# zengyan-97/X2-VLM

Hardware: AMD Instinct MI355X
Metric: image-text pairs/sec (fwd+bwd) X2VLM-base 224px bs=64/GPU (higher is better)
Workload: dtype bf16

## Files before the change

### include/x2vlm_hip.h

```cpp
#ifndef X2VLM_HIP_H
#define X2VLM_HIP_H
#include <stdint.h>
#ifdef __cplusplus
extern "C" {
#endif

const char* x2_last_error(void);
int x2_abi_version(void);
int x2_device_cus(void);
int x2_tune(int key, int value);
int x2_tune_get(int key);

int x2_gemm_nt(const void* A, const void* B, void* C, int M, int N, int K, int lda, int ldb, int ldc,
               const float* bias, const float* gamma, const float* resid, int ldr, void* aux, int ldaux,
               int act, int out_f32, unsigned drop_thr16, unsigned drop_seed, float drop_scale, const unsigned* drop_epoch,
               const float* rowscale, float* colsum, void* stream);

int x2_gemm_nt_dgelu_colparts(const void* A, const void* B, void* C, int M, int N, int K, int lda, int ldb, int ldc,
                              const void* aux, int ldaux, float* colparts, int* nrows_out, void* stream);
int x2_gemm_nt_splitk(const void* A, const void* B, float* C, int M, int N, int K, int lda, int ldb, int ldc,
                      int slices, float* ws, long ws_floats, void* stream);

int x2_gemm_tn_grouped(const int64_t* problems, int count, int accumulate, int split, float* ws, long ws_floats,
                       void* stream);

typedef struct X2AttnArgs {
  const void *Q, *K, *V, *O, *dO;
  void *Out, *dQ, *dK, *dV, *dS;
  float *LSE, *Delta;
  long q_bs, q_rs, k_bs, k_rs, v_bs, v_rs, o_bs, o_rs;
  long dq_bs, dq_rs, dk_bs, dk_rs, dv_bs, dv_rs, do_bs, do_rs;
  int B, Bkv, H, Lq, Lk;
  float scale;
  const float* bias;  int bias_ld;
  const float* biasT; int biasT_ld;
  const float* mask;  int mask_ld;
  const int* kv_idx;
  const int* seq_off; const int* seq_ids;
  int ds_ld;
  unsigned drop_thr16, drop_seed; float drop_scale;
  int dbg;
  int head_dim;
  const unsigned* drop_epoch;
  int grid_nx, grid_ny, grid_nz, grid_map;
  int phase;
  float* ws; long ws_floats;
  float* colsum_ws;
} X2AttnArgs;
int x2_attn_fwd(const X2AttnArgs* args, void* stream);
int x2_attn_bwd(const X2AttnArgs* args, void* stream);
int x2_attn_bwd_one_pass(const X2AttnArgs* args);

int x2_layernorm_fwd(const float* x, const float* w, const float* b, void* y_bf16, float* y_f32, float* mean,
                     float* rstd, int rows, int D, float eps, int period, unsigned drop_thr16, unsigned drop_seed,
                     float drop_scale, const unsigned* drop_epoch, void* stream);
int x2_layernorm_bwd(const void* dy , int dy_is_bf16, const float* x, const float* mean, const float* rstd, const float* w,
                     const float* dres, float* dx, void* dx_bf16, float* dw, float* db, float* dcol, int rows, int D,
// ... 129 lines not shown
```

### x2-vlm_amd/_lib.py

```python
import contextlib
import ctypes as C
import os

import torch

_HERE = os.path.dirname(os.path.abspath(__file__))
LIB_PATH = os.environ.get("X2VLM_HIP_LIB") or os.path.join(_HERE, "libx2vlm_hip.so")

P, I, L, F, U = C.c_void_p, C.c_int, C.c_long, C.c_float, C.c_uint


class AttnArgs(C.Structure):
    _fields_ = [(n, P) for n in ("Q", "K", "V", "O", "dO", "Out", "dQ", "dK", "dV", "dS", "LSE", "Delta")] + \
               [(n, L) for n in ("q_bs", "q_rs", "k_bs", "k_rs", "v_bs", "v_rs", "o_bs", "o_rs",
                                 "dq_bs", "dq_rs", "dk_bs", "dk_rs", "dv_bs", "dv_rs", "do_bs", "do_rs")] + \
               [(n, I) for n in ("B", "Bkv", "H", "Lq", "Lk")] + [("scale", F)] + \
               [("bias", P), ("bias_ld", I), ("biasT", P), ("biasT_ld", I), ("mask", P), ("mask_ld", I),
                ("kv_idx", P), ("seq_off", P), ("seq_ids", P), ("ds_ld", I),
                ("drop_thr16", C.c_uint), ("drop_seed", C.c_uint), ("drop_scale", F), ("dbg", I), ("head_dim", I), ("drop_epoch", P),
                ("grid_nx", I), ("grid_ny", I), ("grid_nz", I), ("grid_map", I),
                ("phase", I), ("ws", P), ("ws_floats", L), ("colsum_ws", P)]


_SIGS = {
    "x2_gemm_nt": [P, P, P, I, I, I, I, I, I, P, P, P, I, P, I, I, I, U, U, F, P, P, P, P],
    "x2_gemm_nt_splitk": [P, P, P, I, I, I, I, I, I, I, P, L, P],
    "x2_gemm_nt_dgelu_colparts": [P, P, P, I, I, I, I, I, I, P, I, P, C.POINTER(I), P],
    "x2_gemm_tn_grouped": [P, I, I, I, P, L, P],
    "x2_attn_fwd": [C.POINTER(AttnArgs), P],
    "x2_attn_bwd": [C.POINTER(AttnArgs), P],
    "x2_layernorm_fwd": [P, P, P, P, P, P, P, I, I, F, I, U, U, F, P, P],
    "x2_layernorm_bwd": [P, I, P, P, P, P, P, P, P, P, P, P, I, I, I, U, U, F, U, U, F, P, P, I, I, P, P],
    "x2_colsum_bf16": [P, P, I, I, I, P, I, P],
    "x2_reduce_partials": [P, I, I, I, P, P, P, P],
    "x2_reduce_partials_multi": [P, I, P],
    "x2_cast_transpose_multi": [P, I, P],
    "x2_copy_f32_multi": [P, I, P],
    "x2_layerscale_finish": [P, I, P],
    "x2_rowscale_cast_colsum": [P, P, P, P, I, I, P, I, P],
    "x2_cast_bf16": [P, P, L, P],
    "x2_cast_transpose_bf16": [P, P, P, I, I, I, P],
    "x2_patchify": [P, P, I, I, I, P],
    "x2_assemble_tokens": [P, P, P, I, I, I, P],
    "x2_assemble_tokens_bwd": [P, P, P, I, I, I, P],
    "x2_pool_tokens": [P, P, I, I, I, I, P],
    "x2_relpos_bias": [P, P, P, P, P, I, I, I, I, F, P],
    "x2_relpos_bias_bwd": [P, P, P, P, I, I, I, I, I, P, I, P],
    "x2_embed_fwd": [P, P, P, P, P, I, I, I, P],
    "x2_embed_bwd": [P, P, P, P, P, I, I, I, P, P],
    "x2_gather_rows": [P, P, P, P, I, L, P],
    "x2_scatter_rows": [P, P, P, I, I, L, P],
    "x2_linear_f32": [P, P, P, P, P, F, I, I, I, L, L, L, L, L, I, I, P, P],
    "x2_l2norm": [P, P, P, I, I, I, P],
    "x2_ce_fwd": [P, L, P, I, I, P, P, P, P],
    "x2_ce_bwd": [P, L, P, P, P, P, F, I, I, P, P, L, P],
    "x2_mlm_ce_fwd": [P, P, P, P, I, I, I, I, I, I, P, P, P],
    "x2_ce_combine": [P, I, P, P, I, P, P, P, P],
    "x2_mlm_ce_bwd": [P, P, P, P, P, P, P, F, I, I, I, I, I, I, P, L, P],
    "x2_sample_negatives": [P, I, P, P, P, P],
    "x2_mask_tokens": [P, P, I, I, P, I, P, I, U, P, C.c_double, I, C.c_double, I, I, L, L, L, L, P, P, P, P],
    "x2_additive_mask": [P, P, I, I, I, F, P],
# ... 13 lines not shown
    "x2_mlm_ls_fwd": [P, P, P, P, L, I, I, I, I, I, I, P, P, P, P, P],
    "x2_ls_combine": [P, P, I, P, P, P, P, I, I, L, F, P, P, P, P],
    "x2_mlm_ls_bwd": [P, P, P, P, P, P, P, P, F, F, L, I, I, I, I, I, I, P, L, P],
    "x2_attn_decode": [P, I, P, P, I, I, I, I, I, I, F, P],
    "x2_beam_gather": [P, P, P, I, I, I, I, I, P],
    "x2_logprob_topk": [P, I, I, I, P, I, I, I, I, I, I, P, P, P, P],
    "x2_answer_topk": [P, I, I, I, P, I, I, P, P, P],
    "x2_vqa_candidates": [P, P, P, I, I, I, I, L, P, P, P, P, I, P],
    "x2_vqa_rerank": [P, I, P, P, I, I, P, P, P, P],
    "x2_bbox_loss_fwd": [P, P, P, I, P, P, P],
    "x2_bbox_loss_bwd": [P, P, P, P, P, P, P, I, P, P],
    "x2_grounding_iou": [P, P, P, I, P, P, P],
    "x2_cls_tail_fwd": [P, I, P, P, P, P, P, I, I, I, F, P, P, P, P, P],
    "x2_cls_tail_bwd": [P, I, P, P, P, P, P, P, P, P, P, I, I, I, P, I, P, P, P, P, P],
    "x2_cls_accuracy": [P, P, I, I, P, P, P],
    "x2_lngelu_fwd": [P, I, P, P, I, I, F, P, I, P, P],
    "x2_lngelu_bwd": [P, I, P, I, P, P, P, I, I, P, I, P, P, P],
    "x2_soft_ce_fwd": [P, I, I, I, P, P, P, I, P, P, P, P],
    "x2_kl_ce_fwd": [P, I, P, I, I, I, P, P, P, P, P],
    "x2_soft_ce_bwd": [P, I, I, I, P, P, P, P, P, P, P, I, P, I, I, P],
    "x2_kl_ce_bwd": [P, I, P, I, I, I, P, P, P, P, I, P, I, I, P],
    "x2_cls_accuracy_rows": [P, I, P, I, I, P, P, P, P],
}
_COMM_SIGS = {
    "x2_comm_unique_id": [P],
    "x2_comm_init": [P, I, I, C.POINTER(P)],
    "x2_comm_info": [P, C.POINTER(I), C.POINTER(I)],
    "x2_comm_allreduce_bucket": [P, P, L, I, I, P, P],
    "x2_comm_allgather": [P, P, P, L, I, P, P],
    "x2_comm_broadcast": [P, P, L, I, I, P, P],
    "x2_comm_destroy": [P],
}
EXPORTS = sorted(list(_SIGS) + list(_COMM_SIGS) + ["x2_last_error", "x2_abi_version", "x2_device_cus", "x2_tune", "x2_tune_get",
                                                         "x2_attn_bwd_one_pass"])

_lib = None


class X2HipError(RuntimeError):
    pass


def lib():
    global _lib
    if _lib is None:
        if not os.path.exists(LIB_PATH):
            raise X2HipError("HIP extension %s not built: run `python -c 'import __graft_entry__ as g; g.build()'`"
                             % LIB_PATH)
        try:
            h = C.CDLL(LIB_PATH)
        except OSError as e:
            raise X2HipError("cannot load %s: %s" % (LIB_PATH, e))
        for name, sig in list(_SIGS.items()) + list(_COMM_SIGS.items()):
            fn = getattr(h, name)
            fn.argtypes, fn.restype = sig, I
        h.x2_last_error.restype = C.c_char_p
        h.x2_abi_version.restype = I
        h.x2_device_cus.restype = I
        h.x2_tune.argtypes, h.x2_tune.restype = [I, I], I
        h.x2_tune_get.argtypes, h.x2_tune_get.restype = [I], I
        h.x2_attn_bwd_one_pass.argtypes, h.x2_attn_bwd_one_pass.restype = [C.POINTER(AttnArgs)], I
        for kv in filter(None, os.environ.get("X2_TUNE", "").split(",")):
            k, v = kv.split("=")
            set_tune(int(k), int(v), h)
        _lib = h
    return _lib


def set_tune(key, value, h=None):
    h = lib() if h is None else h
    if h.x2_tune(key, value) != 0:
        raise X2HipError("x2_tune(%d, %d): %s" % (key, value, h.x2_last_error().decode()))


@contextlib.contextmanager
def tuned(knobs):
    h = lib()
    with contextlib.ExitStack() as undo:
        for key, value in knobs.items():
            prev = h.x2_tune_get(key)
            if prev == -1:
                raise X2HipError("x2_tune_get(%d): no such key" % key)
            if prev != value:
                set_tune(key, value, h)
                undo.callback(set_tune, key, prev, h)
        yield


_get_device = torch._C._cuda_getDevice if hasattr(torch._C, "_cuda_getDevice") else None
_get_raw_stream = getattr(torch._C, "_cuda_getCurrentRawStream", None)


def raw_stream():
    return _get_raw_stream(_get_device())
# ... 12 lines not shown
```

### x2-vlm_amd/csrc/gemm.hip

```cpp
#include "x2_common.h"
#include <type_traits>

#define BM 128
#define BN 128
#define BK 64
#define TILE_BYTES (128 * 128)
#define STAGE_BYTES (2 * TILE_BYTES)
#define GEMM_LDS_BYTES (2 * STAGE_BYTES)

struct GemmNT {
  const bf16_t* A; const bf16_t* B; void* C;
  const float* bias; const float* gamma; const float* resid; bf16_t* aux;
  int M, N, K;
  int lda, ldb, ldc, ldr, ldaux;
  int act;
  int out_f32;
  int group_m;
  DropSpec drop;
  const uint32_t* drop_epoch;
  const float* rowscale;
  float* colsum;
  int dbg;
  int ksplit;
  const long* ce_labels;
  const float* ce_lse;
  const float* ce_g;
  const float* ce_stat;
  float* ce_part;
  float* ce_zlab;
  float ce_gscale;
  int ce_C;
  float* ce_sumz;
  float* ce_zign;
  long ce_ignore;
// ... 1163 lines not shown
  launch_nt_ce(p, 9, (hipStream_t)stream);
  return x2_check_launch("x2_mlm_ce_bwd");
}
extern "C" int x2_mlm_ls_fwd(const void* X, const void* E, const float* bias, const long* labels, long ignore, int R, int Vp, int V, int Hd,
                             int ldx, int lde, float* part, float* sumz, float* zlab, float* zign, void* stream) {
  X2_REQUIRE(X && E && labels && part && sumz && zlab && zign, "x2_mlm_ls_fwd: null argument");
  X2_REQUIRE(mlm_ce_shapes_ok(R, Vp, V, Hd, ldx, lde) && V > 2 && ignore >= 0 && ignore < V,
             "x2_mlm_ls_fwd: R=%d Vp=%d V=%d Hd=%d ldx=%d lde=%d ignore=%ld", R, Vp, V, Hd, ldx, lde, ignore);
  GemmNT p{(const bf16_t*)X, (const bf16_t*)E, nullptr, bias, nullptr, nullptr, nullptr, R, Vp, Hd, ldx, lde, Vp, 0, 0, 0, 0,
           g_tune[0] > 0 ? g_tune[0] : 8, DropSpec{0u, 0u, 1.f}, nullptr, nullptr, nullptr, 0, 0,
           labels, nullptr, nullptr, nullptr, part, zlab, 1.f, V, sumz, zign, ignore, 0.f, nullptr};
  launch_nt_ce(p, 11, (hipStream_t)stream);
  return x2_check_launch("x2_mlm_ls_fwd");
}
extern "C" int x2_mlm_ls_bwd(const void* X, const void* E, const float* bias, const long* labels, const float* w, const float* lse, const float* g,
                             const float* stat, float gscale, float ls, long ignore, int R, int Vp, int V, int Hd, int ldx, int lde, void* dl_bf16,
                             long ldd, void* stream) {
  X2_REQUIRE(X && E && labels && w && lse && g && stat && dl_bf16, "x2_mlm_ls_bwd: null argument");
  X2_REQUIRE(mlm_ce_shapes_ok(R, Vp, V, Hd, ldx, lde) && ldd >= Vp && ldd % 8 == 0 && V > 2 && ignore >= 0 && ignore < V && ls >= 0.f && ls <= 1.f,
             "x2_mlm_ls_bwd: R=%d Vp=%d V=%d Hd=%d ldd=%ld ignore=%ld", R, Vp, V, Hd, ldd, ignore);
  GemmNT p{(const bf16_t*)X, (const bf16_t*)E, dl_bf16, bias, nullptr, nullptr, nullptr, R, Vp, Hd, ldx, lde, (int)ldd, 0, 0, 0, 0,
           g_tune[0] > 0 ? g_tune[0] : 8, DropSpec{0u, 0u, 1.f}, nullptr, nullptr, nullptr, 0, 0,
           labels, lse, g, stat, nullptr, nullptr, gscale, V, nullptr, nullptr, ignore, ls, w};
  launch_nt_ce(p, 12, (hipStream_t)stream);
  return x2_check_launch("x2_mlm_ls_bwd");
}

struct TNProblem {
  const bf16_t* A; const bf16_t* B; float* C;
  int Mc, N, K;
  int lda, ldb, ldc;
  int n_ld, k_ld;
  int tile_begin, tiles_k;
};
struct GemmTNGroup { TNProblem p[8]; int count; int accumulate; };

__device__ __forceinline__ int tn_f(int r) { return (r & 3) | (((r >> 3) & 1) << 2); }

__global__ __launch_bounds__(256, 2) void gemm_tn_kernel(GemmTNGroup g) {
  extern __shared__ __attribute__((aligned(16))) char smem[];
  const int tid = threadIdx.x, lane = tid & 63;
  const int wave = __builtin_amdgcn_readfirstlane(tid >> 6);
  const int wn = wave >> 1, wk = wave & 1;
  int t = xcd_remap(blockIdx.x, gridDim.x);
  int pi = 0;
#pragma unroll
  for (int i = 1; i < 8; ++i) if (i < g.count && t >= g.p[i].tile_begin) pi = i;
  const TNProblem p = g.p[pi];
  t -= p.tile_begin;
  int tnn, tkk;
  tile_coords(t, (p.N + 127) / 128, p.tiles_k, 8, tnn, tkk);
  const int n0 = tnn * 128, k0 = tkk * 128;
  const int steps = (p.Mc + BK - 1) / BK;
  const int per = (steps + gridDim.y - 1) / gridDim.y;
  const int s_begin = blockIdx.y * per, s_end = min(steps, s_begin + per);
  if (s_begin >= s_end) return;

  const bf16_t* srcA[4]; const bf16_t* srcB[4]; int rowq[4];
#pragma unroll
  for (int i = 0; i < 4; ++i) {
    const int q = i * 256 + tid, row = q >> 4, c = (q & 15) ^ (tn_f(row) << 1);
    int ca = n0 + c * 8; ca = ca <= p.n_ld - 8 ? ca : p.n_ld - 8;
    int cb = k0 + c * 8; cb = cb <= p.k_ld - 8 ? cb : p.k_ld - 8;
    rowq[i] = row;
    srcA[i] = p.A + (size_t)row * p.lda + ca;
    srcB[i] = p.B + (size_t)row * p.ldb + cb;
  }
  auto stage = [&](int s, int buf) {
    char* base = smem + buf * STAGE_BYTES;
    const int mbase = s * BK;
    if (mbase + BK <= p.Mc) {
#pragma unroll
      for (int i = 0; i < 4; ++i) {
        glds16(srcA[i] + (size_t)mbase * p.lda, base + (i * 256 + wave * 64) * 16);
        glds16(srcB[i] + (size_t)mbase * p.ldb, base + TILE_BYTES + (i * 256 + wave * 64) * 16);
      }
    } else {
#pragma unroll
      for (int i = 0; i < 4; ++i) {
        u32x4 va = u32x4{0, 0, 0, 0}, vb = u32x4{0, 0, 0, 0};
        if (mbase + rowq[i] < p.Mc) {
          va = *reinterpret_cast<const u32x4*>(srcA[i] + (size_t)mbase * p.lda);
// ... 52 lines not shown
    const int n = n0 + wn * 64 + j * 16 + fi;
    if (n >= p.N) continue;
#pragma unroll
    for (int i = 0; i < 4; ++i) {
      const int k = k0 + wk * 64 + i * 16 + fg * 4;
      if (k >= p.K) continue;
      float* dst = p.C + (size_t)n * p.ldc + k;
      if (atomic) {
#pragma unroll
        for (int r = 0; r < 4; ++r) atomicAdd(dst + r, acc[i][j][r]);
      } else if (g.accumulate) {
        float4 o = *reinterpret_cast<float4*>(dst);
        o.x += acc[i][j][0]; o.y += acc[i][j][1]; o.z += acc[i][j][2]; o.w += acc[i][j][3];
        *reinterpret_cast<float4*>(dst) = o;
      } else {
        *reinterpret_cast<float4*>(dst) = float4{acc[i][j][0], acc[i][j][1], acc[i][j][2], acc[i][j][3]};
      }
    }
  }
}

#define T2_HALF 16384
#define T2_LDS_BYTES (8 * T2_HALF)
__device__ __attribute__((aligned(16))) const uint32_t x2_zero_chunk[4] = {0u, 0u, 0u, 0u};
template <bool RAG>
__global__ __launch_bounds__(512) void gemm_tn256_kernel(GemmTNGroup g, float* ws, int total_tiles) {
  extern __shared__ __attribute__((aligned(16))) char smem[];
  const int tid = threadIdx.x, lane = tid & 63;
  const int wave = __builtin_amdgcn_readfirstlane(tid >> 6);
  const int wr = wave >> 2, wc = wave & 3;
  const int tile = xcd_remap(blockIdx.x, gridDim.x);
  int pi = 0;
#pragma unroll
  for (int i = 1; i < 8; ++i) if (i < g.count && tile >= g.p[i].tile_begin) pi = i;
  const TNProblem p = g.p[pi];
  int tnn, tkk;
  tile_coords(tile - p.tile_begin, (p.N + 255) / 256, p.tiles_k, 4, tnn, tkk);
  const int n0 = tnn * 256, k0 = tkk * 256;
  const int steps = (p.Mc + BK - 1) / BK, rag = p.Mc % BK;
  const int s_begin = (int)((long)steps * blockIdx.y / gridDim.y), s_end = (int)((long)steps * (blockIdx.y + 1) / gridDim.y);
  const int nk = s_end - s_begin;
  const int last_rel = (RAG && rag != 0 && s_end == steps) ? nk - 1 : -1;
  const bf16_t* const zsrc = reinterpret_cast<const bf16_t*>(x2_zero_chunk);
  const bool oob0 = (tid >> 4) >= rag, oob1 = ((512 + tid) >> 4) >= rag;

  const bf16_t* srcA[2][2]; const bf16_t* srcB[2][2];
#pragma unroll
  for (int h = 0; h < 2; ++h)
#pragma unroll
    for (int i = 0; i < 2; ++i) {
      const int q = i * 512 + tid, row = q >> 4, c = (q & 15) ^ (tn_f(row) << 1);
      int ca = n0 + h * 128 + c * 8; ca = ca <= p.n_ld - 8 ? ca : p.n_ld - 8;
      int cb = k0 + h * 128 + c * 8; cb = cb <= p.k_ld - 8 ? cb : p.k_ld - 8;
      srcA[h][i] = p.A + ((size_t)s_begin * BK + row) * p.lda + ca;
      srcB[h][i] = p.B + ((size_t)s_begin * BK + row) * p.ldb + cb;
    }
  const size_t stepA = (size_t)BK * p.lda, stepB = (size_t)BK * p.ldb;
  auto issue = [&](int kt, auto slot) {
    constexpr int S = decltype(slot)::value;
    char* base = smem + ((kt & 1) * 4 + S) * T2_HALF + wave * 1024;
    const bool z = RAG && kt == last_rel;
    if constexpr (S < 2) {
      glds16(z && oob0 ? zsrc : srcA[S][0] + kt * stepA, base);
      glds16(z && oob1 ? zsrc : srcA[S][1] + kt * stepA, base + 8192);
    } else {
      glds16(z && oob0 ? zsrc : srcB[S - 2][0] + kt * stepB, base);
      glds16(z && oob1 ? zsrc : srcB[S - 2][1] + kt * stepB, base + 8192);
    }
  };
  using S0 = std::integral_constant<int, 0>; using S1 = std::integral_constant<int, 1>;
// ... 68 lines not shown
  int kt = 0;
  for (; kt + 2 < nk; ++kt) ktile(kt, std::true_type{}, std::true_type{});
  if (kt + 1 < nk) { ktile(kt, std::true_type{}, std::false_type{}); ++kt; }
  ktile(kt, std::false_type{}, std::false_type{});

  if (gridDim.y > 1) {
    float* dst = ws + ((size_t)blockIdx.y * total_tiles + tile) * 65536 + (size_t)wave * 8192 + lane * 4;
#pragma unroll
    for (int i = 0; i < 4; ++i)
#pragma unroll
      for (int j = 0; j < 8; ++j)
        *reinterpret_cast<float4*>(dst + (i * 8 + j) * 256) = float4{acc[i][j][0], acc[i][j][1], acc[i][j][2], acc[i][j][3]};
    return;
  }
#pragma unroll
  for (int j = 0; j < 8; ++j) {
    const int n = n0 + wr * 128 + j * 16 + fi;
    if (n >= p.N) continue;
#pragma unroll
    for (int i = 0; i < 4; ++i) {
      const int k = k0 + wc * 64 + i * 16 + fg * 4;
      if (k >= p.K) continue;
      float* dst = p.C + (size_t)n * p.ldc + k;
      float4 o = float4{acc[i][j][0], acc[i][j][1], acc[i][j][2], acc[i][j][3]};
      if (g.accumulate) { const float4 c = *reinterpret_cast<float4*>(dst); o.x += c.x; o.y += c.y; o.z += c.z; o.w += c.w; }
      *reinterpret_cast<float4*>(dst) = o;
    }
  }
}
__global__ __launch_bounds__(256) void gemm_tn256_reduce_kernel(GemmTNGroup g, const float* __restrict__ ws, int total_tiles, int split) {
  const int tile = blockIdx.x >> 6;
  int pi = 0;
#pragma unroll
  for (int i = 1; i < 8; ++i) if (i < g.count && tile >= g.p[i].tile_begin) pi = i;
  const TNProblem p = g.p[pi];
  int tnn, tkk;
  tile_coords(tile - p.tile_begin, (p.N + 255) / 256, p.tiles_k, 4, tnn, tkk);
  const int e = (blockIdx.x & 63) * 256 + threadIdx.x;
  const int lane = e & 63, ij = (e >> 6) & 31, wave = e >> 11;
  const int i = ij >> 3, j = ij & 7, fi = lane & 15, fg = lane >> 4, wr = wave >> 2, wc = wave & 3;
  const int n = tnn * 256 + wr * 128 + j * 16 + fi, k = tkk * 256 + wc * 64 + i * 16 + fg * 4;
  const float* src = ws + (size_t)tile * 65536 + (size_t)e * 4;
  float4 o = *reinterpret_cast<const float4*>(src);
  for (int s_ = 1; s_ < split; ++s_) {
    const float4 v = *reinterpret_cast<const float4*>(src + (size_t)s_ * total_tiles * 65536);
    o.x += v.x; o.y += v.y; o.z += v.z; o.w += v.w;
  }
  if (n >= p.N || k >= p.K) return;
  float* dst = p.C + (size_t)n * p.ldc + k;
  if (g.accumulate) { const float4 c = *reinterpret_cast<float4*>(dst); o.x += c.x; o.y += c.y; o.z += c.z; o.w += c.w; }
  *reinterpret_cast<float4*>(dst) = o;
}

extern "C" int x2_gemm_tn_grouped(const int64_t* problems, int count, int accumulate, int split, float* ws, long ws_floats,
                                  void* stream) {
  X2_REQUIRE(count >= 1 && count <= 8, "x2_gemm_tn_grouped: count=%d not in [1,8]", count);
  X2_REQUIRE(split >= 0, "x2_gemm_tn_grouped: split=%d", split);
  GemmTNGroup g; g.count = count; g.accumulate = accumulate;
  int tiles = 0, tiles256 = 0, min_steps = 1 << 30;
  bool big = g_tune[5] != 1;
  for (int i = 0; i < count; ++i) {
    const int64_t* q = problems + i * 11;
    TNProblem& p = g.p[i];
    p.A = (const bf16_t*)q[0]; p.B = (const bf16_t*)q[1]; p.C = (float*)q[2];
    p.Mc = (int)q[3]; p.N = (int)q[4]; p.K = (int)q[5]; p.lda = (int)q[6]; p.ldb = (int)q[7]; p.ldc = (int)q[8];
    p.n_ld = (int)q[9]; p.k_ld = (int)q[10];
    X2_REQUIRE(p.Mc > 0 && p.N > 0 && p.K > 0, "x2_gemm_tn_grouped[%d]: empty problem", i);
    X2_REQUIRE(p.K % 4 == 0 && p.ldc % 4 == 0, "x2_gemm_tn_grouped[%d]: K, ldc must be multiples of 4", i);
    X2_REQUIRE(p.lda % 8 == 0 && p.ldb % 8 == 0 && p.n_ld % 8 == 0 && p.k_ld % 8 == 0 && p.n_ld >= 8 && p.k_ld >= 8,
               "x2_gemm_tn_grouped[%d]: rows must be 16-byte granular", i);
    X2_REQUIRE(p.n_ld <= p.lda && p.k_ld <= p.ldb, "x2_gemm_tn_grouped[%d]: n_ld/k_ld exceed leading dims", i);
    tiles += ((p.N + 127) / 128) * ((p.K + 127) / 128);
    tiles256 += ((p.N + 255) / 256) * ((p.K + 255) / 256);
    const int steps_i = (p.Mc + BK - 1) / BK;
    min_steps = steps_i < min_steps ? steps_i : min_steps;
  }
  if (g_tune[5] != 2 && tiles256 < 24 && !(split > 1 && ws)) big = false;
  if (big) {
    int t = 0;
    for (int i = 0; i < count; ++i) { g.p[i].tile_begin = t; g.p[i].tiles_k = (g.p[i].K + 255) / 256; t += ((g.p[i].N + 255) / 256) * g.p[i].tiles_k; }
    const int cus = x2_cus();
    int sp = split;
    if (sp == 0) {
      double best = -1.0; sp = 1;
      for (int c = 1; c <= 4 && min_steps / c >= 16; ++c) {
        const long blocks = (long)t * c;
        const double fill = (double)blocks / (double)(((blocks + cus - 1) / cus) * cus);
        if (fill > best + 0.03) { best = fill; sp = c; }
      }
    }
    while (sp > 1 && (sp > min_steps || !ws || (long)sp * t * 65536 > ws_floats)) --sp;
    static bool attr = false;
    if (!attr) {
      (void)hipFuncSetAttribute(reinterpret_cast<const void*>(gemm_tn256_kernel<false>), hipFuncAttributeMaxDynamicSharedMemorySize, T2_LDS_BYTES);
      (void)hipFuncSetAttribute(reinterpret_cast<const void*>(gemm_tn256_kernel<true>), hipFuncAttributeMaxDynamicSharedMemorySize, T2_LDS_BYTES);
      attr = true;
    }
    bool ragged = false;
    for (int i = 0; i < count; ++i) ragged = ragged || (g.p[i].Mc % BK != 0);
    if (ragged) hipLaunchKernelGGL(gemm_tn256_kernel<true>, dim3(t, sp), dim3(512), T2_LDS_BYTES, (hipStream_t)stream, g, ws, t);
    else hipLaunchKernelGGL(gemm_tn256_kernel<false>, dim3(t, sp), dim3(512), T2_LDS_BYTES, (hipStream_t)stream, g, ws, t);
    if (sp > 1) hipLaunchKernelGGL(gemm_tn256_reduce_kernel, dim3(t * 64), dim3(256), 0, (hipStream_t)stream, g, ws, t, sp);
    return x2_check_launch("x2_gemm_tn_grouped");
  }
  if (split == 0) split = 1;
  X2_REQUIRE(split == 1 || accumulate, "x2_gemm_tn_grouped: split>1 on the 128x128 kernel adds atomically: pass accumulate=1 and a defined C");
  int t = 0;
  for (int i = 0; i < count; ++i) { g.p[i].tile_begin = t; g.p[i].tiles_k = (g.p[i].K + 127) / 128; t += ((g.p[i].N + 127) / 128) * g.p[i].tiles_k; }
  hipLaunchKernelGGL(gemm_tn_kernel, dim3(t, split), dim3(256), GEMM_LDS_BYTES, (hipStream_t)stream, g);
  return x2_check_launch("x2_gemm_tn_grouped");
}
```

### x2-vlm_amd/engine.py

```python
import itertools
import math
import weakref

import torch

from . import kernels as K
from ._lib import raw_stream

BF16, F32 = torch.bfloat16, torch.float32



_SERIAL = itertools.count(1)


def _tok(w):
    t = w.__dict__.get("_x2_serial")
    if t is None:
        t = w.__dict__["_x2_serial"] = next(_SERIAL)
    return t


class TScale:

# ... 255 lines not shown
            return
        self.pending.append((G, tn, deferred))
        self.extra += list(param_only)
        self.fin += list(finish)
        if len(self.pending) == 2:
            self.flush()

    def flush(self):
        if self.pending:
            entries, self.pending = self.pending, []
            extra, self.extra = self.extra, []
            fin, self.fin = self.fin, []
            self._launch(entries, extra, fin)

    @staticmethod
    def _launch(entries, extra=(), fin=()):
        deferred = [d for _, _, ds in entries for d in (ds or ())]
        tn = [pr for _, t, _ in entries for pr in t]

        def work():
            if deferred:
                K.reduce_partials_multi(deferred)
            K.gemm_tn_grouped(tn)
            if fin:
                K.layerscale_finish(fin)
        if WGRAD_QUEUE is not None:
            tn_a = [tuple(pr[:2]) + (pr[2].detach(),) + tuple(pr[3:]) for pr in tn]
            def_a = [(ws, nblk, nk, width, tuple(None if o is None else o.detach() for o in outs)) for ws, nblk, nk, width, outs in deferred]
            fin_a = [tuple(t.detach() if (torch.is_tensor(t) and not isinstance(t, torch.nn.Parameter)) else t for t in it) for it in fin]
            pubs = [(G.flat, G.key, list(G.params)) for G, _, _ in entries]

            extra = list(extra)

            def later():
                for fn in extra:
                    fn()
                if def_a:
                    K.reduce_partials_multi(def_a)
                K.gemm_tn_grouped(tn_a)
                if fin_a:
                    K.layerscale_finish(fin_a)
                if GRAD_READY_HOOK is not None:
                    for flat, key, params in pubs:
                        GRAD_READY_HOOK(flat, key, None, params)
            later.params = set(id(p_) for _, _, ps in pubs for p_ in ps)
            for fn in WGRAD_QUEUE:
                if getattr(fn, "params", set()) & later.params:
                    raise RuntimeError("engine.WGRAD_QUEUE: a layer ran twice in one pass; its weight gradients cannot be deferred "
                                       "(graph.SegmentedStep: defer_tail_wgrad, the deferred vision stages)")
            WGRAD_QUEUE.append(later)
            return
        assert not extra, "param_only closures are only collected while WGRAD_QUEUE is set"
        keep = [t for pr in tn for t in pr[:2]] + [G.flat for G, _, _ in entries] + [d[0] for d in deferred]
        done = SIDE.launch(work, keep)
        for G, _, _ in entries:
            G.publish(done)


def _param_only(po, fn, src, dst):
    if WGRAD_QUEUE is not None:
        dst_a = dst.detach()
        po.append(lambda: fn(src, dst_a))
    else:
        fn(src, dst)


def _finish_layer_backward(G, tn):
    deferred, K.DEFERRED = K.DEFERRED, None
    _LayerPairs._launch([(G, tn, deferred)])


WGRAD_QUEUE = None
GRAD_READY_HOOK = None
STAGE_CALLS = {}


def _count_call(key):
    STAGE_CALLS[key] = STAGE_CALLS.get(key, 0) + 1


def _mask_pad(add_mask, Lk):
    S = add_mask.shape[0]
    out = torch.zeros(S, K.round_up(Lk, 64), device=add_mask.device, dtype=F32)
    out[:, :Lk] = add_mask
    return out



def vision_param_names(depth, lo=0, hi=None):
# ... 703 lines not shown
```

### x2-vlm_amd/graph.py

```python
import contextlib
import gc
import os

import torch

from . import kernels as K
from ._lib import tuned


class GraphedStep:
    def __init__(self, fn, warmup=2, enabled=True, verbose=False):
        self.fn, self.graph, self.out = fn, None, None
        self._grads = []
        self.stream = torch.cuda.Stream()
        self.mode = "eager"
        self.error = None
        self._epoch = None
        if not enabled or os.environ.get("X2_GRAPH", "1") == "0":
            return
        from . import engine
        if K.DROP_EPOCH is None:
            K.DROP_EPOCH = torch.zeros(1, dtype=torch.int32, device="cuda")
        self._epoch = K.DROP_EPOCH
        side_rule, engine.SIDE.only_from = engine.SIDE.only_from, self.stream.cuda_stream
# ... 317 lines not shown
        t["loss"] = {k: v.detach() for k, v in loss.items()}

    def _backward(self, losses):
        tot = self.total_loss(losses)
        if torch.is_tensor(tot) and tot.requires_grad:
            tot.backward()

    def _s_vision_bwd(self, ci=0):
        if ci == 0:
            ie_out, _, full_out = self.t["vis"]
            pairs = [(ie_out, self.t["ie"].grad)]
            if full_out is not None:
                pairs.append((full_out, self.t["full"].grad))
        else:
            x, leaf = self.t["vmid"][len(self.vcuts) - ci]
            pairs = [(x, leaf.grad)]
        pairs = [(o, g) for o, g in pairs if g is not None]
        if pairs:
            torch.autograd.backward([o for o, _ in pairs], [g for _, g in pairs])

    def _s_vision_wgrad(self, ci):
        work = self._vq.pop(ci, None)
        self._held.append(work)
        for fn in work or ():
            fn()

    def _s_text_bwd(self):
        if self.t["both_leaf"].grad is not None:
            torch.autograd.backward([self.t["both"]], [self.t["both_leaf"].grad])

    def _s_tail_wgrad(self):
        work, self._queue = self._queue, None
        self._held.append(work)
        for fn in work or ():
            fn()

    def _run(self, mode):
        eng, A, Bs = self.engine, self.sA, self.sB
        pa = pb = None
        if mode == "capture":
            pa, pb = self._pools
        if mode != "replay":
            eng.SIDE.enabled = False
            eng.TIE_WORD_GRAD = True
            if self.recast_weights:
                eng.BANK.invalidate()
            else:
                eng.BANK.backward_seen = False
            for p in self.params:
                p.grad = None
        with torch.cuda.stream(A):
            self._epoch.add_(1)
        Bs.wait_stream(A)
        self._seg(mode, "T", Bs, self._s_text, pb)
        if self.recast_weights:
            self._seg(mode, "P", Bs, self._s_prefetch, pb)
        self._seg(mode, "V", A, self._s_vision, pa)
        A.wait_stream(Bs)
        self._seg(mode, "F1", A, self._s_feat, pa)
        with torch.cuda.stream(A):
            self._gather()
        if mode != "replay":
            eng.WGRAD_QUEUE = [] if self.defer_tail_wgrad else None
            eng.AUX.enabled, eng.AUX.only_from, eng.AUX.auto = self.aux_overlap, self.sA.cuda_stream, self.aux_auto
        try:
            self._seg(mode, "F2", A, self._s_loss, pa)
        finally:
            eng.AUX.enabled, eng.AUX.only_from, eng.AUX.auto = False, None, False
# ... 351 lines not shown
```

### x2-vlm_amd/kernels.py

```python
import ctypes as C

import torch

from . import _lib
from ._lib import AttnArgs, call, ptr, raw_stream

BF16, F32 = torch.bfloat16, torch.float32


GEMM_TIMER = None


class _timed:

    def __init__(self, flops, name="gemm_nt"):
        self.flops = flops
        self.name = name

    def __enter__(self):
        if GEMM_TIMER is not None:
            self.a = torch.cuda.Event(enable_timing=True)
            self.b = torch.cuda.Event(enable_timing=True)
            self.a.record()

# ... 118 lines not shown

def gemm_nt_dgelu_colsum(A, B, pre, colsum):
    assert A.dtype == BF16 and B.dtype == BF16 and A.shape[1] == B.shape[1] and pre.dtype == BF16
    M, K = A.shape
    N = B.shape[0]
    assert pre.shape == (M, N) and colsum.dtype == F32 and colsum.numel() == N
    out = torch.empty(M, N, device=A.device, dtype=BF16)
    ws, defer = _ws_and_defer(A.device, 2 * ((M + 63) // 64) * N)
    nrows = C.c_int(0)
    with _timed(2.0 * M * N * K):
        call("x2_gemm_nt_dgelu_colparts", ptr(A), ptr(B), ptr(out), M, N, K, _rows(A), _rows(B), _rows(out), ptr(pre), _rows(pre),
             ptr(ws), C.byref(nrows))
    if defer:
        DEFERRED.append((ws, nrows.value, 1, N, (colsum,)))
    else:
        reduce_partials(ws, nrows.value, 1, N, (colsum,))
    return out


def gemm_nt_splitk(A, B, out=None, slices=0):
    assert A.dtype == BF16 and B.dtype == BF16 and A.shape[1] == B.shape[1]
    M, K = A.shape
    N = B.shape[0]
    if out is None:
        out = torch.empty(M, N, device=A.device, dtype=F32)
    assert out.shape == (M, N) and out.dtype == F32
    ws = workspace(A.device, min(32, max(1, K // 64)) * M * N)
    with _timed(2.0 * M * N * K):
        call("x2_gemm_nt_splitk", ptr(A), ptr(B), ptr(out), M, N, K, _rows(A), _rows(B), _rows(out), slices, ptr(ws), ws.numel())
    return out


def gemm_tn_grouped(problems, accumulate=False, split=0):
    rows = []
    for pr in problems:
        dY, X, dW = pr[:3]
        assert dY.dtype == BF16 and X.dtype == BF16 and dW.dtype == F32 and dY.shape[0] == X.shape[0]
        N, K = dW.shape
        n_ld, k_ld = (pr[3], pr[4]) if len(pr) == 5 else (dY.shape[1], X.shape[1])
        assert dY.shape[1] >= N or n_ld >= N
        rows.append([dY.data_ptr(), X.data_ptr(), dW.data_ptr(), dY.shape[0], N, K, _rows(dY), _rows(X), _rows(dW),
                     n_ld, k_ld])
    dev = problems[0][0].device
    for i in range(0, len(rows), 8):
        chunk = rows[i:i + 8]
        arr = (C.c_int64 * (11 * len(chunk)))(*[v for r in chunk for v in r])
        tiles256 = sum(((r[4] + 255) // 256) * ((r[5] + 255) // 256) for r in chunk)
        want = (split if split else 4) * tiles256 * 65536
        ws = workspace(dev, want) if split != 1 else None
        with _timed(sum(2.0 * r[3] * r[4] * r[5] for r in chunk), "gemm_tn"):
            call("x2_gemm_tn_grouped", arr, len(chunk), 1 if accumulate else 0, split, ptr(ws), 0 if ws is None else ws.numel())



def _attn_args(q, k, v, B, Bkv, H, Lq, Lk, scale, bias=None, biasT=None, mask=None, kv_idx=None, seq_off=None,
               seq_ids=None, drop=NO_DROP, head_dim=64, bias_log2=False):
    a = AttnArgs()
    a.Q, a.q_bs, a.q_rs = q
    a.K, a.k_bs, a.k_rs = k
    a.V, a.v_bs, a.v_rs = v
    a.B, a.Bkv, a.H, a.Lq, a.Lk, a.scale = B, Bkv, H, Lq, Lk, scale
    a.head_dim = head_dim
    a.dbg = 16 if bias_log2 else 0
    a.drop_thr16, a.drop_seed, a.drop_scale = drop[:3]
    a.drop_epoch = ptr(drop[3])
    if bias is not None:
        assert bias.dtype == F32 and bias.dim() == 3 and bias.is_contiguous()
        a.bias, a.bias_ld = bias.data_ptr(), bias.shape[2]
    if biasT is not None:
        assert biasT.dtype == F32 and biasT.dim() == 3 and biasT.is_contiguous()
        a.biasT, a.biasT_ld = biasT.data_ptr(), biasT.shape[2]
    if mask is not None:
        assert mask.dtype == F32 and mask.dim() == 2 and mask.is_contiguous() and mask.shape[0] == B
        a.mask, a.mask_ld = mask.data_ptr(), mask.shape[1]
    if kv_idx is not None:
        assert kv_idx.dtype == torch.int32 and kv_idx.numel() == B
        a.kv_idx = kv_idx.data_ptr()
    if seq_off is not None:
        assert seq_off.dtype == torch.int32 and seq_ids.dtype == torch.int32
        a.seq_off, a.seq_ids = seq_off.data_ptr(), seq_ids.data_ptr()
    return a


def view3(t, B, L, col0=0):
# ... 810 lines not shown
```

Baseline: 2941.

## Pack queued weight-gradient GEMMs into CU-aligned multi-layer grouped launches

Adds a planner that concatenates the weight-gradient TN GEMM tiles of all queued layers and cuts them into launches whose tile counts are multiples of the CU count. Only the remainder launch uses split-K, and per-layer finish hooks fire once their last tile launch is issued. The goal is to cut per-layer launch overhead and partial-wave tail waste in the backward tail. In exchange, a tile window can now span problems (up to 32 entries per group), the host must replan on every call, and the Python side now issues several launches with callbacks.

```diff
diff --git a/include/x2vlm_hip.h b/include/x2vlm_hip.h
--- a/include/x2vlm_hip.h
+++ b/include/x2vlm_hip.h
@@ -23,6 +23,10 @@
 
 int x2_gemm_tn_grouped(const int64_t* problems, int count, int accumulate, int split, float* ws, long ws_floats,
                        void* stream);
+int x2_tn_plan(const int64_t* shapes, int count, int cus, long ws_floats, int* windows, int max_windows, int* launches, int max_launches,
+               int* n_windows, int* n_launches);
+int x2_gemm_tn_queue(const int64_t* problems, int count, int accumulate, float* ws, long ws_floats, int first_launch, int n_launches,
+                     void* stream);
 
 typedef struct X2AttnArgs {
   const void *Q, *K, *V, *O, *dO;
diff --git a/x2-vlm_amd/_lib.py b/x2-vlm_amd/_lib.py
--- a/x2-vlm_amd/_lib.py
+++ b/x2-vlm_amd/_lib.py
@@ -27,6 +27,7 @@
     "x2_gemm_nt_splitk": [P, P, P, I, I, I, I, I, I, I, P, L, P],
     "x2_gemm_nt_dgelu_colparts": [P, P, P, I, I, I, I, I, I, P, I, P, C.POINTER(I), P],
     "x2_gemm_tn_grouped": [P, I, I, I, P, L, P],
+    "x2_gemm_tn_queue": [P, I, I, P, L, I, I, P],
     "x2_attn_fwd": [C.POINTER(AttnArgs), P],
     "x2_attn_bwd": [C.POINTER(AttnArgs), P],
     "x2_layernorm_fwd": [P, P, P, P, P, P, P, I, I, F, I, U, U, F, P, P],
@@ -106,7 +107,7 @@
     "x2_comm_destroy": [P],
 }
 EXPORTS = sorted(list(_SIGS) + list(_COMM_SIGS) + ["x2_last_error", "x2_abi_version", "x2_device_cus", "x2_tune", "x2_tune_get",
-                                                         "x2_attn_bwd_one_pass"])
+                                                         "x2_attn_bwd_one_pass", "x2_tn_plan"])
 
 _lib = None
 
@@ -134,6 +135,7 @@
         h.x2_tune.argtypes, h.x2_tune.restype = [I, I], I
         h.x2_tune_get.argtypes, h.x2_tune_get.restype = [I], I
         h.x2_attn_bwd_one_pass.argtypes, h.x2_attn_bwd_one_pass.restype = [C.POINTER(AttnArgs)], I
+        h.x2_tn_plan.argtypes, h.x2_tn_plan.restype = [P, I, I, L, P, I, P, I, C.POINTER(I), C.POINTER(I)], I
         for kv in filter(None, os.environ.get("X2_TUNE", "").split(",")):
             k, v = kv.split("=")
             set_tune(int(k), int(v), h)
diff --git a/x2-vlm_amd/csrc/gemm.hip b/x2-vlm_amd/csrc/gemm.hip
--- a/x2-vlm_amd/csrc/gemm.hip
+++ b/x2-vlm_amd/csrc/gemm.hip
@@ -1,5 +1,7 @@
 #include "x2_common.h"
+#include <algorithm>
 #include <type_traits>
+#include <vector>
 
 #define BM 128
 #define BN 128
@@ -1229,8 +1231,10 @@
   int lda, ldb, ldc;
   int n_ld, k_ld;
   int tile_begin, tiles_k;
+  int tile_first;
 };
-struct GemmTNGroup { TNProblem p[8]; int count; int accumulate; };
+#define TN_MAX_ENTRIES 32
+struct GemmTNGroup { TNProblem p[TN_MAX_ENTRIES]; int count; int accumulate; };
 
 __device__ __forceinline__ int tn_f(int r) { return (r & 3) | (((r >> 3) & 1) << 2); }
 
@@ -1242,9 +1246,9 @@
   int t = xcd_remap(blockIdx.x, gridDim.x);
   int pi = 0;
 #pragma unroll
-  for (int i = 1; i < 8; ++i) if (i < g.count && t >= g.p[i].tile_begin) pi = i;
+  for (int i = 1; i < TN_MAX_ENTRIES; ++i) if (i < g.count && t >= g.p[i].tile_begin) pi = i;
   const TNProblem p = g.p[pi];
-  t -= p.tile_begin;
+  t -= p.tile_begin - p.tile_first;
   int tnn, tkk;
   tile_coords(t, (p.N + 127) / 128, p.tiles_k, 8, tnn, tkk);
   const int n0 = tnn * 128, k0 = tkk * 128;
@@ -1363,10 +1367,10 @@
   const int tile = xcd_remap(blockIdx.x, gridDim.x);
   int pi = 0;
 #pragma unroll
-  for (int i = 1; i < 8; ++i) if (i < g.count && tile >= g.p[i].tile_begin) pi = i;
+  for (int i = 1; i < TN_MAX_ENTRIES; ++i) if (i < g.count && tile >= g.p[i].tile_begin) pi = i;
   const TNProblem p = g.p[pi];
   int tnn, tkk;
-  tile_coords(tile - p.tile_begin, (p.N + 255) / 256, p.tiles_k, 4, tnn, tkk);
+  tile_coords(tile - p.tile_begin + p.tile_first, (p.N + 255) / 256, p.tiles_k, 4, tnn, tkk);
   const int n0 = tnn * 256, k0 = tkk * 256;
   const int steps = (p.Mc + BK - 1) / BK, rag = p.Mc % BK;
   const int s_begin = (int)((long)steps * blockIdx.y / gridDim.y), s_end = (int)((long)steps * (blockIdx.y + 1) / gridDim.y);
@@ -1501,10 +1505,10 @@
   const int tile = blockIdx.x >> 6;
   int pi = 0;
 #pragma unroll
-  for (int i = 1; i < 8; ++i) if (i < g.count && tile >= g.p[i].tile_begin) pi = i;
+  for (int i = 1; i < TN_MAX_ENTRIES; ++i) if (i < g.count && tile >= g.p[i].tile_begin) pi = i;
   const TNProblem p = g.p[pi];
   int tnn, tkk;
-  tile_coords(tile - p.tile_begin, (p.N + 255) / 256, p.tiles_k, 4, tnn, tkk);
+  tile_coords(tile - p.tile_begin + p.tile_first, (p.N + 255) / 256, p.tiles_k, 4, tnn, tkk);
   const int e = (blockIdx.x & 63) * 256 + threadIdx.x;
   const int lane = e & 63, ij = (e >> 6) & 31, wave = e >> 11;
   const int i = ij >> 3, j = ij & 7, fi = lane & 15, fg = lane >> 4, wr = wave >> 2, wc = wave & 3;
@@ -1521,25 +1525,55 @@
   *reinterpret_cast<float4*>(dst) = o;
 }
 
+static int tn_parse(const char* who, const int64_t* q, int i, TNProblem& p) {
+  p.A = (const bf16_t*)q[0]; p.B = (const bf16_t*)q[1]; p.C = (float*)q[2];
+  p.Mc = (int)q[3]; p.N = (int)q[4]; p.K = (int)q[5]; p.lda = (int)q[6]; p.ldb = (int)q[7]; p.ldc = (int)q[8];
+  p.n_ld = (int)q[9]; p.k_ld = (int)q[10];
+  p.tile_begin = 0; p.tiles_k = 0; p.tile_first = 0;
+  X2_REQUIRE(p.Mc > 0 && p.N > 0 && p.K > 0, "%s[%d]: empty problem", who, i);
+  X2_REQUIRE(p.K % 4 == 0 && p.ldc % 4 == 0, "%s[%d]: K, ldc must be multiples of 4", who, i);
+  X2_REQUIRE(p.lda % 8 == 0 && p.ldb % 8 == 0 && p.n_ld % 8 == 0 && p.k_ld % 8 == 0 && p.n_ld >= 8 && p.k_ld >= 8,
+             "%s[%d]: rows must be 16-byte granular", who, i);
+  X2_REQUIRE(p.n_ld <= p.lda && p.k_ld <= p.ldb, "%s[%d]: n_ld/k_ld exceed leading dims", who, i);
+  return X2_OK;
+}
+static int tn_split_rule(int t, int min_steps, int cus, int split, bool have_ws, long ws_floats) {
+  int sp = split;
+  if (sp == 0) {
+    double best = -1.0; sp = 1;
+    for (int c = 1; c <= 4 && min_steps / c >= 16; ++c) {
+      const long blocks = (long)t * c;
+      const double fill = (double)blocks / (double)(((blocks + cus - 1) / cus) * cus);
+      if (fill > best + 0.03) { best = fill; sp = c; }
+    }
+  }
+  while (sp > 1 && (sp > min_steps || !have_ws || (long)sp * t * 65536 > ws_floats)) --sp;
+  return sp;
+}
+static void tn256_launch(const GemmTNGroup& g, int t, int sp, float* ws, hipStream_t stream) {
+  static bool attr = false;
+  if (!attr) {
+    (void)hipFuncSetAttribute(reinterpret_cast<const void*>(gemm_tn256_kernel<false>), hipFuncAttributeMaxDynamicSharedMemorySize, T2_LDS_BYTES);
+    (void)hipFuncSetAttribute(reinterpret_cast<const void*>(gemm_tn256_kernel<true>), hipFuncAttributeMaxDynamicSharedMemorySize, T2_LDS_BYTES);
+    attr = true;
+  }
+  bool ragged = false;
+  for (int i = 0; i < g.count; ++i) ragged = ragged || (g.p[i].Mc % BK != 0);
+  if (ragged) hipLaunchKernelGGL(gemm_tn256_kernel<true>, dim3(t, sp), dim3(512), T2_LDS_BYTES, stream, g, ws, t);
+  else hipLaunchKernelGGL(gemm_tn256_kernel<false>, dim3(t, sp), dim3(512), T2_LDS_BYTES, stream, g, ws, t);
+  if (sp > 1) hipLaunchKernelGGL(gemm_tn256_reduce_kernel, dim3(t * 64), dim3(256), 0, stream, g, ws, t, sp);
+}
+
 extern "C" int x2_gemm_tn_grouped(const int64_t* problems, int count, int accumulate, int split, float* ws, long ws_floats,
                                   void* stream) {
   X2_REQUIRE(count >= 1 && count <= 8, "x2_gemm_tn_grouped: count=%d not in [1,8]", count);
   X2_REQUIRE(split >= 0, "x2_gemm_tn_grouped: split=%d", split);
-  GemmTNGroup g; g.count = count; g.accumulate = accumulate;
-  int tiles = 0, tiles256 = 0, min_steps = 1 << 30;
+  GemmTNGroup g{}; g.count = count; g.accumulate = accumulate;
+  int tiles256 = 0, min_steps = 1 << 30;
   bool big = g_tune[5] != 1;
   for (int i = 0; i < count; ++i) {
-    const int64_t* q = problems + i * 11;
     TNProblem& p = g.p[i];
-    p.A = (const bf16_t*)q[0]; p.B = (const bf16_t*)q[1]; p.C = (float*)q[2];
-    p.Mc = (int)q[3]; p.N = (int)q[4]; p.K = (int)q[5]; p.lda = (int)q[6]; p.ldb = (int)q[7]; p.ldc = (int)q[8];
-    p.n_ld = (int)q[9]; p.k_ld = (int)q[10];
-    X2_REQUIRE(p.Mc > 0 && p.N > 0 && p.K > 0, "x2_gemm_tn_grouped[%d]: empty problem", i);
-    X2_REQUIRE(p.K % 4 == 0 && p.ldc % 4 == 0, "x2_gemm_tn_grouped[%d]: K, ldc must be multiples of 4", i);
-    X2_REQUIRE(p.lda % 8 == 0 && p.ldb % 8 == 0 && p.n_ld % 8 == 0 && p.k_ld % 8 == 0 && p.n_ld >= 8 && p.k_ld >= 8,
-               "x2_gemm_tn_grouped[%d]: rows must be 16-byte granular", i);
-    X2_REQUIRE(p.n_ld <= p.lda && p.k_ld <= p.ldb, "x2_gemm_tn_grouped[%d]: n_ld/k_ld exceed leading dims", i);
-    tiles += ((p.N + 127) / 128) * ((p.K + 127) / 128);
+    if (int rc = tn_parse("x2_gemm_tn_grouped", problems + i * 11, i, p)) return rc;
     tiles256 += ((p.N + 255) / 256) * ((p.K + 255) / 256);
     const int steps_i = (p.Mc + BK - 1) / BK;
     min_steps = steps_i < min_steps ? steps_i : min_steps;
@@ -1548,28 +1582,8 @@
   if (big) {
     int t = 0;
     for (int i = 0; i < count; ++i) { g.p[i].tile_begin = t; g.p[i].tiles_k = (g.p[i].K + 255) / 256; t += ((g.p[i].N + 255) / 256) * g.p[i].tiles_k; }
-    const int cus = x2_cus();
-    int sp = split;
-    if (sp == 0) {
-      double best = -1.0; sp = 1;
-      for (int c = 1; c <= 4 && min_steps / c >= 16; ++c) {
-        const long blocks = (long)t * c;
-        const double fill = (double)blocks / (double)(((blocks + cus - 1) / cus) * cus);
-        if (fill > best + 0.03) { best = fill; sp = c; }
-      }
-    }
-    while (sp > 1 && (sp > min_steps || !ws || (long)sp * t * 65536 > ws_floats)) --sp;
-    static bool attr = false;
-    if (!attr) {
-      (void)hipFuncSetAttribute(reinterpret_cast<const void*>(gemm_tn256_kernel<false>), hipFuncAttributeMaxDynamicSharedMemorySize, T2_LDS_BYTES);
-      (void)hipFuncSetAttribute(reinterpret_cast<const void*>(gemm_tn256_kernel<true>), hipFuncAttributeMaxDynamicSharedMemorySize, T2_LDS_BYTES);
-      attr = true;
-    }
-    bool ragged = false;
-    for (int i = 0; i < count; ++i) ragged = ragged || (g.p[i].Mc % BK != 0);
-    if (ragged) hipLaunchKernelGGL(gemm_tn256_kernel<true>, dim3(t, sp), dim3(512), T2_LDS_BYTES, (hipStream_t)stream, g, ws, t);
-    else hipLaunchKernelGGL(gemm_tn256_kernel<false>, dim3(t, sp), dim3(512), T2_LDS_BYTES, (hipStream_t)stream, g, ws, t);
-    if (sp > 1) hipLaunchKernelGGL(gemm_tn256_reduce_kernel, dim3(t * 64), dim3(256), 0, (hipStream_t)stream, g, ws, t, sp);
+    const int sp = tn_split_rule(t, min_steps, x2_cus(), split, ws != nullptr, ws_floats);
+    tn256_launch(g, t, sp, ws, (hipStream_t)stream);
     return x2_check_launch("x2_gemm_tn_grouped");
   }
   if (split == 0) split = 1;
@@ -1579,3 +1593,101 @@
   hipLaunchKernelGGL(gemm_tn_kernel, dim3(t, split), dim3(256), GEMM_LDS_BYTES, (hipStream_t)stream, g);
   return x2_check_launch("x2_gemm_tn_grouped");
 }
+
+struct TNWindow { int launch, problem, first, tiles; };
+struct TNPlan { std::vector<TNWindow> win; std::vector<int> split, remainder; };
+static void tn_plan(const int64_t* shapes, int stride, int count, int cus, long ws_floats, TNPlan& plan) {
+  std::vector<int> tiles(count), steps(count);
+  long total = 0;
+  for (int i = 0; i < count; ++i) {
+    const int64_t* q = shapes + (size_t)i * stride;
+    tiles[i] = (int)(((q[1] + 255) / 256) * ((q[2] + 255) / 256));
+    steps[i] = (int)((q[0] + BK - 1) / BK);
+    total += tiles[i];
+  }
+  const long main_tiles = total / cus * cus;
+  int launch = -1;
+  auto emit = [&](long from, long to, bool rem, bool dry) -> long {
+    if (!dry) { ++launch; plan.split.push_back(1); plan.remainder.push_back(rem ? 1 : 0); }
+    long begin = 0, pos = from;
+    int entries = 0;
+    for (int i = 0; i < count && pos < to && entries < TN_MAX_ENTRIES; begin += tiles[i], ++i) {
+      if (pos >= begin + tiles[i]) continue;
+      const int first = (int)(pos - begin), n = (int)std::min<long>(tiles[i] - first, to - pos);
+      if (!dry) plan.win.push_back(TNWindow{launch, i, first, n});
+      ++entries; pos += n;
+    }
+    return pos;
+  };
+  for (long pos = 0; pos < main_tiles;) {
+    long end = emit(pos, main_tiles, false, true);
+    if (end < main_tiles && end / cus * cus > pos) end = end / cus * cus;
+    pos = emit(pos, end, false, false);
+  }
+  for (long pos = main_tiles; pos < total;) pos = emit(pos, total, true, false);
+  for (int l = 0; l <= launch; ++l) {
+    if (!plan.remainder[l]) continue;
+    int t = 0, min_steps = 1 << 30;
+    for (const TNWindow& w : plan.win) if (w.launch == l) { t += w.tiles; min_steps = std::min(min_steps, steps[w.problem]); }
+    plan.split[l] = tn_split_rule(t, min_steps, cus, 0, ws_floats > 0, ws_floats);
+  }
+}
+
+extern "C" int x2_tn_plan(const int64_t* shapes, int count, int cus, long ws_floats, int* windows, int max_windows, int* launches,
+                          int max_launches, int* n_windows, int* n_launches) {
+  X2_REQUIRE(shapes && count >= 1 && n_windows && n_launches, "x2_tn_plan: null argument or count=%d", count);
+  for (int i = 0; i < count; ++i)
+    X2_REQUIRE(shapes[3 * i] > 0 && shapes[3 * i + 1] > 0 && shapes[3 * i + 2] > 0 && shapes[3 * i] < (1L << 31) && shapes[3 * i + 1] < (1L << 24) &&
+               shapes[3 * i + 2] < (1L << 24), "x2_tn_plan[%d]: Mc, N, K out of range", i);
+  if (cus <= 0) cus = x2_cus();
+  TNPlan plan;
+  tn_plan(shapes, 3, count, cus, ws_floats, plan);
+  *n_windows = (int)plan.win.size(); *n_launches = (int)plan.split.size();
+  X2_REQUIRE((windows || max_windows == 0) && (launches || max_launches == 0), "x2_tn_plan: null output");
+  if (max_windows == 0 && max_launches == 0) return X2_OK;
+  X2_REQUIRE(*n_windows <= max_windows && *n_launches <= max_launches, "x2_tn_plan: %d windows, %d launches exceed the room given (%d, %d)",
+             *n_windows, *n_launches, max_windows, max_launches);
+  for (size_t w = 0; w < plan.win.size(); ++w) {
+    windows[4 * w] = plan.win[w].launch; windows[4 * w + 1] = plan.win[w].problem; windows[4 * w + 2] = plan.win[w].first; windows[4 * w + 3] = plan.win[w].tiles;
+  }
+  for (size_t l = 0; l < plan.split.size(); ++l) { launches[2 * l] = plan.split[l]; launches[2 * l + 1] = plan.remainder[l]; }
+  return X2_OK;
+}
+
+extern "C" int x2_gemm_tn_queue(const int64_t* problems, int count, int accumulate, float* ws, long ws_floats, int first_launch,
+                                int n_launches, void* stream) {
+  X2_REQUIRE(problems && count >= 1 && first_launch >= 0 && n_launches >= 0, "x2_gemm_tn_queue: count=%d first_launch=%d n_launches=%d", count,
+             first_launch, n_launches);
+  std::vector<TNProblem> pr(count);
+  long tiles256 = 0;
+  for (int i = 0; i < count; ++i) {
+    if (int rc = tn_parse("x2_gemm_tn_queue", problems + (size_t)i * 11, i, pr[i])) return rc;
+    tiles256 += (long)((pr[i].N + 255) / 256) * ((pr[i].K + 255) / 256);
+  }
+  if (g_tune[5] == 1 || (g_tune[5] != 2 && tiles256 < 24)) {
+    X2_REQUIRE(first_launch == 0, "x2_gemm_tn_queue: first_launch=%d of a one-launch plan", first_launch);
+    for (int i = 0; i < count; i += 8)
+      if (int rc = x2_gemm_tn_grouped(problems + (size_t)i * 11, std::min(8, count - i), accumulate, 0, ws, ws_floats, stream)) return rc;
+    return X2_OK;
+  }
+  if (!ws) ws_floats = 0;
+  TNPlan plan;
+  tn_plan(problems + 3, 11, count, x2_cus(), ws_floats, plan);
+  const int nl = (int)plan.split.size();
+  X2_REQUIRE(first_launch < nl, "x2_gemm_tn_queue: first_launch=%d of %d launches", first_launch, nl);
+  const int end = n_launches == 0 ? nl : std::min(nl, first_launch + n_launches);
+  size_t w = 0;
+  for (int l = 0; l < end; ++l) {
+    GemmTNGroup g{}; g.count = 0; g.accumulate = accumulate;
+    int t = 0;
+    for (; w < plan.win.size() && plan.win[w].launch == l; ++w) {
+      TNProblem& p = g.p[g.count++];
+      p = pr[plan.win[w].problem];
+      p.tile_begin = t; p.tiles_k = (p.K + 255) / 256; p.tile_first = plan.win[w].first;
+      t += plan.win[w].tiles;
+    }
+    if (l < first_launch) continue;
+    tn256_launch(g, t, plan.split[l], ws, (hipStream_t)stream);
+  }
+  return x2_check_launch("x2_gemm_tn_queue");
+}
diff --git a/x2-vlm_amd/engine.py b/x2-vlm_amd/engine.py
--- a/x2-vlm_amd/engine.py
+++ b/x2-vlm_amd/engine.py
@@ -311,17 +311,24 @@
 
             extra = list(extra)
 
-            def later():
+            def pre():
                 for fn in extra:
                     fn()
                 if def_a:
                     K.reduce_partials_multi(def_a)
-                K.gemm_tn_grouped(tn_a)
+
+            def post():
                 if fin_a:
                     K.layerscale_finish(fin_a)
                 if GRAD_READY_HOOK is not None:
                     for flat, key, params in pubs:
                         GRAD_READY_HOOK(flat, key, None, params)
+
+            def later():
+                pre()
+                K.gemm_tn_grouped(tn_a)
+                post()
+            later.pre, later.tn, later.post = pre, tn_a, post
             later.params = set(id(p_) for _, _, ps in pubs for p_ in ps)
             for fn in WGRAD_QUEUE:
                 if getattr(fn, "params", set()) & later.params:
@@ -334,6 +341,23 @@
         done = SIDE.launch(work, keep)
         for G, _, _ in entries:
             G.publish(done)
+
+
+def run_wgrad_queue(work):
+    work = list(work or ())
+    if len(work) < 2:
+        for fn in work:
+            fn()
+        return
+    for fn in work:
+        assert fn.tn, "engine.run_wgrad_queue: a queued layer without weight-gradient problems"
+        fn.pre()
+    tn, ends = [], {}
+    for fn in work:
+        tn += fn.tn
+        ends[len(tn) - 1] = fn.post
+    K.gemm_tn_queue(tn, done=lambda i: ends.pop(i)() if i in ends else None)
+    assert not ends, "engine.run_wgrad_queue: %d layers were never completed" % len(ends)
 
 
 def _param_only(po, fn, src, dst):
diff --git a/x2-vlm_amd/graph.py b/x2-vlm_amd/graph.py
--- a/x2-vlm_amd/graph.py
+++ b/x2-vlm_amd/graph.py
@@ -373,8 +373,7 @@
     def _s_tail_wgrad(self):
         work, self._queue = self._queue, None
         self._held.append(work)
-        for fn in work or ():
-            fn()
+        self.engine.run_wgrad_queue(work)
 
     def _run(self, mode):
         eng, A, Bs = self.engine, self.sA, self.sB
diff --git a/x2-vlm_amd/kernels.py b/x2-vlm_amd/kernels.py
--- a/x2-vlm_amd/kernels.py
+++ b/x2-vlm_amd/kernels.py
@@ -174,15 +174,7 @@
 
 
 def gemm_tn_grouped(problems, accumulate=False, split=0):
-    rows = []
-    for pr in problems:
-        dY, X, dW = pr[:3]
-        assert dY.dtype == BF16 and X.dtype == BF16 and dW.dtype == F32 and dY.shape[0] == X.shape[0]
-        N, K = dW.shape
-        n_ld, k_ld = (pr[3], pr[4]) if len(pr) == 5 else (dY.shape[1], X.shape[1])
-        assert dY.shape[1] >= N or n_ld >= N
-        rows.append([dY.data_ptr(), X.data_ptr(), dW.data_ptr(), dY.shape[0], N, K, _rows(dY), _rows(X), _rows(dW),
-                     n_ld, k_ld])
+    rows = _tn_rows(problems)
     dev = problems[0][0].device
     for i in range(0, len(rows), 8):
         chunk = rows[i:i + 8]
@@ -192,6 +184,69 @@
         ws = workspace(dev, want) if split != 1 else None
         with _timed(sum(2.0 * r[3] * r[4] * r[5] for r in chunk), "gemm_tn"):
             call("x2_gemm_tn_grouped", arr, len(chunk), 1 if accumulate else 0, split, ptr(ws), 0 if ws is None else ws.numel())
+
+
+_CUS = {}
+
+
+def _device_cus(dev):
+    if dev not in _CUS:
+        _CUS[dev] = (_lib.lib().x2_device_cus() if dev.type == "cuda" else 0) or 256
+    return _CUS[dev]
+
+
+def _tn_rows(problems):
+    rows = []
+    for pr in problems:
+        dY, X, dW = pr[:3]
+        assert dY.dtype == BF16 and X.dtype == BF16 and dW.dtype == F32 and dY.shape[0] == X.shape[0]
+        N, K = dW.shape
+        n_ld, k_ld = (pr[3], pr[4]) if len(pr) == 5 else (dY.shape[1], X.shape[1])
+        assert dY.shape[1] >= N or n_ld >= N
+        rows.append([dY.data_ptr(), X.data_ptr(), dW.data_ptr(), dY.shape[0], N, K, _rows(dY), _rows(X), _rows(dW), n_ld, k_ld])
+    return rows
+
+
+def tn_plan(shapes, cus=0, ws_floats=0):
+    flat = (C.c_int64 * (3 * len(shapes)))(*[int(v) for s in shapes for v in s])
+    nw, nl = C.c_int(0), C.c_int(0)
+    h = _lib.lib()
+
+    def ask(*a):
+        if h.x2_tn_plan(flat, len(shapes), cus, ws_floats, *a, C.byref(nw), C.byref(nl)) != 0:
+            raise RuntimeError("x2_tn_plan: %s" % h.x2_last_error().decode())
+    ask(None, 0, None, 0)
+    win, lau = (C.c_int * (4 * nw.value))(), (C.c_int * (2 * nl.value))()
+    ask(win, nw.value, lau, nl.value)
+    return ([tuple(win[4 * i:4 * i + 4]) for i in range(nw.value)], [tuple(lau[2 * i:2 * i + 2]) for i in range(nl.value)])
+
+
+def gemm_tn_queue(problems, accumulate=False, done=None):
+    rows = _tn_rows(problems)
+    dev = problems[0][0].device
+    arr = (C.c_int64 * (11 * len(rows)))(*[v for r in rows for v in r])
+    tiles = [((r[4] + 255) // 256) * ((r[5] + 255) // 256) for r in rows]
+    want = 4 * min(sum(tiles), max(_device_cus(dev) - 1, 1)) * 65536
+    ws = workspace(dev, want)
+    acc = 1 if accumulate else 0
+    flops = sum(2.0 * r[3] * r[4] * r[5] for r in rows)
+    if done is None or sum(tiles) < 24 or _lib.lib().x2_tune_get(5) == 1:
+        with _timed(flops, "gemm_tn"):
+            call("x2_gemm_tn_queue", arr, len(rows), acc, ptr(ws), want, 0, 0)
+        for i in range(len(rows) if done is not None else 0):
+            done(i)
+        return
+    windows, launches = tn_plan([r[3:6] for r in rows], 0, want)
+    last = {}
+    for launch, prob, _first, _n in windows:
+        last[prob] = launch
+    nxt = 0
+    for l in range(len(launches)):
+        with _timed(flops / len(launches), "gemm_tn"):
+            call("x2_gemm_tn_queue", arr, len(rows), acc, ptr(ws), want, l, 1)
+        while nxt < len(rows) and last[nxt] == l:
+            done(nxt)
+            nxt += 1
 
 
 
```

Result: faster. 2986, median of 6 (+1.5%).
